# meyerls/PEGASUS

Measured on AMD Instinct MI355X. Metric: rendered views/sec (RGB+depth+mask) on 2M-Gaussian scene @800x800, higher is better.
Workload: dtype f32

## Files before the change

### pegasus_amd/csrc/cull.hip.h

```cpp
#pragma once
#include "pgr_common.h"

namespace pgr {

__device__ __forceinline__ float edge_min_q(float A, float B, float C, float r, float d_fixed, float lo, float hi) {
    float t = -(d_fixed * r);
    t = fminf(hi, fmaxf(lo, t));
    return A * d_fixed * d_fixed + 2.0f * B * d_fixed * t + C * t * t;
}

struct CullSplat { float mx, my, A, B, C, rBC, rBA, tau; uint32_t flags; };

__device__ __forceinline__ CullSplat make_cull_splat(float2 xy, float4 co, float rBC, float rBA) {
    CullSplat s;
    s.mx = xy.x; s.my = xy.y; s.A = co.x; s.B = co.y; s.C = co.z;
    s.flags = (co.w < ALPHA_MIN ? 1u : 0u)
            | ((!(co.x > 0.0f) || !(co.z > 0.0f)) ? 2u : 0u);
    s.rBC = rBC;
    s.rBA = rBA;
    const float t = 255.0f * co.w;
    const uint32_t bits = __float_as_uint(t);
    const float e = (float)((int)((bits >> 23) & 0xffu) - 127);
    const float m = __uint_as_float((bits & 0x007fffffu) | 0x3f800000u);
    s.tau = 1.3862944f * (e + (m - 1.0f) + 0.0861f);
    return s;
}

__device__ __forceinline__ CullSplat make_cull_splat(float2 xy, float4 co) {
    return make_cull_splat(xy, co, co.y / co.z, co.y / co.x);
}

__device__ __forceinline__ bool rect_may_contribute(const CullSplat& s, float x0, float y0, float x1, float y1) {
    if (s.flags & 1u) return false;
    if (s.flags & 2u) return true;
    if (s.mx >= x0 && s.mx <= x1 && s.my >= y0 && s.my <= y1) return true;
    const float dx0 = x0 - s.mx, dx1 = x1 - s.mx, dy0 = y0 - s.my, dy1 = y1 - s.my;
    const float dxn = s.mx < x0 ? dx0 : dx1, dyn = s.my < y0 ? dy0 : dy1;
    const float q = fminf(edge_min_q(s.A, s.B, s.C, s.rBC, dxn, dy0, dy1), edge_min_q(s.C, s.B, s.A, s.rBA, dyn, dx0, dx1));
    const float DX = fmaxf(fabsf(dx0), fabsf(dx1)), DY = fmaxf(fabsf(dy0), fabsf(dy1));
    const float M = s.A * DX * DX + 2.0f * fabsf(s.B) * DX * DY + s.C * DY * DY;
    return !(q > s.tau + 0.00001f * M + 0.01f);
}

__device__ __forceinline__ bool tile_may_contribute(const CullSplat& s, int tx, int ty, int W, int H) {
    const float x0 = (float)(tx * TILE), y0 = (float)(ty * TILE);
    const float x1 = fminf(x0 + (float)(TILE - 1), (float)(W - 1));
    const float y1 = fminf(y0 + (float)(TILE - 1), (float)(H - 1));
    return rect_may_contribute(s, x0, y0, x1, y1);
}


}
```

### pegasus_amd/csrc/tilebin.hip.h

```cpp
#pragma once
#include <type_traits>

#include "composite.hip.h"
#include "cull.hip.h"
#include "pgr_common.h"

namespace pgr {

constexpr int BIN_CHUNK = 4096;
#ifndef PGR_BIN_THREADS
#define PGR_BIN_THREADS 512
#endif
constexpr int BIN_THREADS = PGR_BIN_THREADS;
constexpr int BIN_LDS_TILES = 16384;
constexpr int SORT_THREADS = 256;

__device__ __forceinline__ uint2 pack_rect(int minx, int miny, int maxx, int maxy) {
    return make_uint2((uint32_t)minx | ((uint32_t)miny << 16), (uint32_t)maxx | ((uint32_t)maxy << 16));
}

struct BinView {
    const uint2* rects;
    const float4* splats;
    uint32_t* tile_count;
    uint32_t* rel;
    uint2* ranges;
    uint32_t* counters;
    uint2* bucket;
    uint32_t* gauss_sorted;
    uint64_t* alt;
    uint32_t* obj_last;
    int32_t n_env;
    const int32_t* tie_index;
    const uint32_t* tie_inv;
    uint2* records;
};


__device__ __forceinline__ uint32_t dpp_u32(uint32_t old, uint32_t v, int ctrl, int row_mask, bool bound) {
    switch (ctrl) {
        case 0x111: return (uint32_t)__builtin_amdgcn_update_dpp((int)old, (int)v, 0x111, 0xF, 0xF, true);
        case 0x112: return (uint32_t)__builtin_amdgcn_update_dpp((int)old, (int)v, 0x112, 0xF, 0xF, true);
        case 0x114: return (uint32_t)__builtin_amdgcn_update_dpp((int)old, (int)v, 0x114, 0xF, 0xF, true);
        case 0x118: return (uint32_t)__builtin_amdgcn_update_dpp((int)old, (int)v, 0x118, 0xF, 0xF, true);
        case 0x142: return (uint32_t)__builtin_amdgcn_update_dpp((int)old, (int)v, 0x142, 0xA, 0xF, false);
        default:    return (uint32_t)__builtin_amdgcn_update_dpp((int)old, (int)v, 0x143, 0xC, 0xF, false);
    }
}

__device__ __forceinline__ uint32_t wave_inclusive_scan(uint32_t v) {
    v += dpp_u32(0, v, 0x111, 0xF, true);
    v += dpp_u32(0, v, 0x112, 0xF, true);
    v += dpp_u32(0, v, 0x114, 0xF, true);
    v += dpp_u32(0, v, 0x118, 0xF, true);
    v += dpp_u32(0, v, 0x142, 0xA, false);
    v += dpp_u32(0, v, 0x143, 0xC, false);
    return v;
}

__device__ __forceinline__ uint32_t wave_inclusive_max(uint32_t v) {
    v = max(v, dpp_u32(0, v, 0x111, 0xF, true));
    v = max(v, dpp_u32(0, v, 0x112, 0xF, true));
    v = max(v, dpp_u32(0, v, 0x114, 0xF, true));
    v = max(v, dpp_u32(0, v, 0x118, 0xF, true));
    v = max(v, dpp_u32(0, v, 0x142, 0xA, false));
    v = max(v, dpp_u32(0, v, 0x143, 0xC, false));
    return v;
}

constexpr int BIN_STAGE_WORDS = WAVE * 12 + WAVE;
constexpr int BIN_THREADS_SMALL = 1024;
__host__ __device__ inline size_t bin_lds_bytes(int tiles, int threads) {
    return ((size_t)(tiles < BIN_LDS_TILES ? tiles : BIN_LDS_TILES) + 3) / 4 * 16 + (size_t)(threads / WAVE) * BIN_STAGE_WORDS * 4 + 16;
}

struct BinLayers {
    const int32_t* layer_id;
    int32_t layer_tiles;
    int32_t layer_rows;
    int32_t n_layers;
};
constexpr uint32_t VERDICT_WINDOWS = 62;
constexpr uint32_t VERDICT_REGION_WORDS = 192;

template <bool SCATTER, int THREADS>
__global__ __launch_bounds__(THREADS) void bin_kernel(const BinView* __restrict__ views, int n, int grid_x,
                                                          int tiles, int W, int H, const uint32_t* __restrict__ vis,
                                                          int vis_words, int verdict_groups,
                                                          BinLayers layers = BinLayers{nullptr, 0, 0, 0}) {
    extern __shared__ __attribute__((aligned(16))) uint32_t lds[];
    constexpr int BIN_WAVES = THREADS / WAVE;
    const BinView& bv = views[blockIdx.y];
    if (SCATTER && gload(bv.counters + 1)) return;
    const int chunk = blockIdx.x;
    const int begin = chunk * BIN_CHUNK, end = min(n, begin + BIN_CHUNK);
    const int lane = threadIdx.x & (WAVE - 1), wave = threadIdx.x / WAVE;
    const bool layered = layers.layer_id != nullptr;
    const int hist_words = (min(layered ? layers.layer_tiles : tiles, BIN_LDS_TILES) + 3) / 4 * 4;
    float4* const stage = reinterpret_cast<float4*>(lds + hist_words + wave * BIN_STAGE_WORDS);
    uint32_t* const heads = reinterpret_cast<uint32_t*>(stage + WAVE * 3);
    uint32_t* const ctrl = lds + hist_words + BIN_WAVES * BIN_STAGE_WORDS;
    constexpr int GROUPS = BIN_CHUNK / WAVE;
    static_assert(GROUPS == WAVE, "one visibility bit per lane of a wave");
    int pass_first = 0, pass_last = (tiles - 1) / BIN_LDS_TILES;
    if (layered) {
        if (begin >= end) return;
        pass_first = max(1, min(layers.n_layers + 1, (int)gload(layers.layer_id + begin)));
        pass_last = min(layers.n_layers, (int)gload(layers.layer_id + end - 1));
    }
    for (int lp = pass_first; lp <= pass_last; ++lp) {
        const int lo = layered ? (lp - 1) * layers.layer_tiles : lp * BIN_LDS_TILES;
        const int span = layered ? layers.layer_tiles : min(BIN_LDS_TILES, tiles - lo);
        const int row_off = layered ? (lp - 1) * layers.layer_rows : 0;
        for (int t = threadIdx.x; t < span; t += THREADS)
            lds[t] = SCATTER ? gload(bv.ranges + lo + t).x + gload(bv.rel + (size_t)chunk * tiles + lo + t) : 0u;
        if (wave == 0) {
            const int b = begin + lane * WAVE;
            bool visible = b < end;
            if (visible && vis) visible = (vis[(size_t)(b / WAVE) * vis_words + (blockIdx.y >> 5)] >> (blockIdx.y & 31)) & 1u;
            const uint64_t m = __ballot(visible);
            if (lane == 0) { ctrl[0] = 0u; ctrl[1] = (uint32_t)m; ctrl[2] = (uint32_t)(m >> 32); }
        }
        __syncthreads();
        const uint64_t vis_bits = ((uint64_t)ctrl[2] << 32) | ctrl[1];
        auto take_ticket = [&]() {
            for (;;) {
                uint32_t ticket = 0;
                if (lane == 0) ticket = atomicAdd(&ctrl[0], 1u);
                ticket = (uint32_t)__builtin_amdgcn_readfirstlane((int)ticket);
                if (ticket >= (uint32_t)GROUPS || ((vis_bits >> ticket) & 1ull)) return ticket;
            }
        };
        for (uint32_t ticket = take_ticket(); ticket < (uint32_t)GROUPS; ticket = take_ticket()) {
            const int base = begin + (int)ticket * WAVE;
            bool has_region = base / WAVE < verdict_groups;
            if (layered) {
                const int l0 = gload(layers.layer_id + base), l1 = gload(layers.layer_id + min(base + WAVE, end) - 1);
                if (lp < l0 || lp > l1) continue;
                has_region = has_region && l0 == l1;
            }
            uint32_t* const region = reinterpret_cast<uint32_t*>(bv.records) + (size_t)(base / WAVE) * VERDICT_REGION_WORDS;
            uint64_t* const ballots = reinterpret_cast<uint64_t*>(region + WAVE);
            const int i = base + lane;
            const int ic = i < end ? i : end - 1;
            uint2 r = gload(bv.rects + ic);
            float4 q0 = make_float4(0.f, 0.f, 0.f, 0.f), q1 = q0;
            float depth = 0.0f;
            uint64_t my_ballot = 0;
            if (SCATTER && has_region) {
                depth = __uint_as_float(gload(region + lane));
                if (lane < (int)VERDICT_WINDOWS) my_ballot = gload(ballots + lane);
            } else {
                q0 = gload(bv.splats + (size_t)ic * 3);
                q1 = gload(bv.splats + (size_t)ic * 3 + 1);
                if (SCATTER || has_region) depth = gload(reinterpret_cast<const float*>(bv.splats + (size_t)ic * 3 + 2) + 3);
            }
            if (i >= end) r = make_uint2(0u, 0u);
            const int w = (int)(r.y & 0xffff) - (int)(r.x & 0xffff), h = (int)(r.y >> 16) - (int)(r.x >> 16);
            const uint32_t area = (w > 0 && h > 0) ? (uint32_t)(w * h) : 0u;
            const uint32_t incl = wave_inclusive_scan(area);
            const uint32_t excl = incl - area;
            const uint32_t total = (uint32_t)__builtin_amdgcn_readlane((int)incl, WAVE - 1);
            const bool bits = has_region && total <= VERDICT_WINDOWS * (uint32_t)WAVE;
            if (SCATTER && has_region && !bits) {
                q0 = gload(bv.splats + (size_t)ic * 3);
                q1 = gload(bv.splats + (size_t)ic * 3 + 1);
                depth = gload(reinterpret_cast<const float*>(bv.splats + (size_t)ic * 3 + 2) + 3);
            }
            auto walk = [&](auto from_bits_c, auto write_bits_c) {
                constexpr bool FROM_BITS = decltype(from_bits_c)::value, WRITE_BITS = decltype(write_bits_c)::value;
                float4 s0 = make_float4(0.f, 0.f, 0.f, 0.f), s1 = s0, s2 = s0;
                if (area) {
                    uint32_t flags = 0;
                    if (!FROM_BITS) {
                        const CullSplat cs = make_cull_splat(make_float2(q0.x, q0.y), make_float4(q0.z, q0.w, q1.x, q1.y), q1.z, q1.w);
                        s0 = make_float4(cs.mx, cs.my, cs.A, cs.B);
                        s1 = make_float4(cs.C, cs.rBC, cs.rBA, cs.tau);
                        flags = cs.flags;
                    }
                    s2 = make_float4(__uint_as_float(flags | ((uint32_t)w << 2)), __uint_as_float(r.x), 1.0f / (float)w, depth);
                }
                if (!FROM_BITS) { stage[lane * 3 + 0] = s0; stage[lane * 3 + 1] = s1; }
                stage[lane * 3 + 2] = s2;
                __builtin_amdgcn_wave_barrier();
                if (WRITE_BITS && total) gstore(region + lane, __float_as_uint(depth));
                uint32_t carry_key = 0;
                uint32_t it = 0;
                for (uint32_t c0 = 0; c0 < total; c0 += WAVE, ++it) {
                    uint64_t verdicts = ~0ull;
                    if (FROM_BITS) {
                        const uint32_t vlo = (uint32_t)__builtin_amdgcn_readlane((int)(uint32_t)my_ballot, (int)it);
                        const uint32_t vhi = (uint32_t)__builtin_amdgcn_readlane((int)(uint32_t)(my_ballot >> 32), (int)it);
                        verdicts = ((uint64_t)vhi << 32) | vlo;
                    }
                    heads[lane] = 0u;
                    asm volatile("" ::: "memory");
                    if (area && excl - c0 < (uint32_t)WAVE) heads[excl - c0] = ((excl + 1u) << 6) | (uint32_t)lane;
                    asm volatile("" ::: "memory");
                    uint32_t key = wave_inclusive_max(heads[lane]);
                    asm volatile("" ::: "memory");
                    key = key ? key : carry_key;
                    carry_key = (uint32_t)__builtin_amdgcn_readlane((int)key, WAVE - 1);
                    if (FROM_BITS && verdicts == 0ull) continue;
                    const uint32_t c = c0 + (uint32_t)lane;
                    const int g = (int)(key & 63u);
                    const uint32_t k = c - ((key >> 6) - 1u);
                    const float4 o2 = stage[g * 3 + 2];
                    const uint32_t fw = __float_as_uint(o2.x), rlo = __float_as_uint(o2.y);
                    const int ow = (int)(fw >> 2);
                    int ty = (int)(((float)k + 0.5f) * o2.z);
                    int tx = (int)k - ty * ow;
                    if (tx < 0) { --ty; tx += ow; } else if (tx >= ow) { ++ty; tx -= ow; }
                    const int x = (int)(rlo & 0xffff) + tx, y = (int)(rlo >> 16) + ty;
                    const int t = y * grid_x + x - lo;
                    bool pass = c < total && (unsigned)t < (unsigned)span;
                    if (FROM_BITS) {
                        pass = pass && ((verdicts >> lane) & 1ull);
                    } else if (pass) {
                        const float4 o0 = stage[g * 3 + 0], o1 = stage[g * 3 + 1];
                        CullSplat cs;
                        cs.mx = o0.x; cs.my = o0.y; cs.A = o0.z; cs.B = o0.w;
                        cs.C = o1.x; cs.rBC = o1.y; cs.rBA = o1.z; cs.tau = o1.w; cs.flags = fw & 3u;
                        pass = tile_may_contribute(cs, x, y - row_off, W, H);
                    }
                    if (WRITE_BITS) {
                        const uint64_t m = __ballot(pass);
                        if (lane == 0) gstore(ballots + it, m);
                    }
                    if (pass) {
                        const uint32_t slot = atomicAdd(&lds[t], 1u);
                        if (SCATTER) gstore(bv.bucket + slot, make_uint2(__float_as_uint(o2.w), (uint32_t)(base + g)));
                    }
                }
            };
            if (SCATTER) {
                if (bits) walk(std::true_type{}, std::false_type{}); else walk(std::false_type{}, std::false_type{});
            } else {
                if (bits) walk(std::false_type{}, std::true_type{}); else walk(std::false_type{}, std::false_type{});
            }
        }
        __syncthreads();
        if (!SCATTER) {
            for (int t = threadIdx.x; t < span; t += THREADS) {
                const uint32_t cnt = lds[t];
                gstore(bv.rel + (size_t)chunk * tiles + lo + t, cnt ? gatomic_add(bv.tile_count + lo + t, cnt) : 0u);
            }
            __syncthreads();
        }
    }
}

__global__ void invert_tie_index_kernel(int n, const int32_t* __restrict__ tie_index, uint32_t* __restrict__ tie_inv) {
    const int i = blockIdx.x * blockDim.x + threadIdx.x;
    if (i >= n) return;
    const int k = tie_index[i];
    if ((unsigned)k < (unsigned)n) tie_inv[k] = (uint32_t)i;
}

__global__ __launch_bounds__(1024) void tile_scan_kernel(const BinView* __restrict__ views, int tiles,
                                                         uint32_t max_instances, int grid_x,
                                                         uint32_t* __restrict__ order_state, int skip_empty,
                                                         uint32_t* __restrict__ host_status) {
    __shared__ unsigned long long wave_tot[1024 / WAVE];
    __shared__ unsigned long long carry_s;
    __shared__ uint32_t hist[ORDER_BINS];
    __shared__ uint32_t last_s;
    const BinView& bv = views[blockIdx.x];
    const int lane = threadIdx.x & (WAVE - 1), wid = threadIdx.x / WAVE;
    if (threadIdx.x == 0) carry_s = 0;
    if (threadIdx.x < ORDER_BINS) hist[threadIdx.x] = 0;
    __syncthreads();
    for (int base = 0; base < tiles; base += 1024) {
        const int idx = base + threadIdx.x;
        const unsigned long long v = idx < tiles ? (unsigned long long)bv.tile_count[idx] : 0ull;
        unsigned long long s = v;
#pragma unroll
        for (int d = 1; d < WAVE; d <<= 1) {
            const unsigned long long t = __shfl_up(s, d, WAVE);
            if (lane >= d) s += t;
        }
        if (lane == WAVE - 1) wave_tot[wid] = s;
        __syncthreads();
        unsigned long long wave_prefix = 0;
        for (int w = 0; w < wid; ++w) wave_prefix += wave_tot[w];
        const unsigned long long carry = carry_s;
        const unsigned long long excl = carry + wave_prefix + s - v;
        const unsigned long long cap = max_instances;
        if (idx < tiles) {
            const uint2 r = make_uint2((uint32_t)min(excl, cap), (uint32_t)min(excl + v, cap));
            bv.ranges[idx] = r;
            if (order_state && !(skip_empty && r.y == r.x))
                atomicAdd(&hist[xcd_of_tile(idx, grid_x) * ORDER_CLASSES_USED + coarse_class(r.y - r.x)], ITEMS_PER_TILE);
        }
        __syncthreads();
        if (threadIdx.x == 1023) carry_s = carry + wave_prefix + s;
        __syncthreads();
    }
    if (threadIdx.x == 0) {
        const uint32_t total = (uint32_t)min(carry_s, 0xffffffffull);
        const uint32_t over = carry_s > (unsigned long long)max_instances ? 1u : 0u;
        bv.counters[0] = total;
        bv.counters[1] = over;
        if (host_status) {
            host_status[2 * blockIdx.x] = total;
            host_status[2 * blockIdx.x + 1] = over;
            __threadfence_system();
        }
    }
    if (!order_state) return;
    if (gridDim.x == 1) {
        __syncthreads();
        if (threadIdx.x < NUM_XCD) {
            uint32_t acc = 0;
            for (int c = 0; c < ORDER_CLASSES_USED; ++c) {
                gstore(order_state + threadIdx.x * ORDER_CLASSES_USED + c, acc);
                acc += hist[threadIdx.x * ORDER_CLASSES_USED + c];
            }
        }
        return;
    }
    if (threadIdx.x < ORDER_BINS && hist[threadIdx.x]) gatomic_add(order_state + threadIdx.x, hist[threadIdx.x]);
    __threadfence();
    __syncthreads();
    if (threadIdx.x == 0) last_s = gatomic_add(order_state + ORDER_DONE_WORD, 1u) == gridDim.x - 1u ? 1u : 0u;
    __syncthreads();
    if (!last_s) return;
    __threadfence();
    if (threadIdx.x < NUM_XCD) {
        uint32_t acc = 0;
        for (int c = 0; c < ORDER_CLASSES_USED; ++c) {
            const uint32_t v = gatomic_load(order_state + threadIdx.x * ORDER_CLASSES_USED + c);
            gstore(order_state + threadIdx.x * ORDER_CLASSES_USED + c, acc);
            acc += v;
        }
    }
}


constexpr uint64_t KEY_INF = ~0ull;

__device__ __forceinline__ uint32_t key_to_pos(const uint32_t* __restrict__ inv, uint32_t tk) { return inv ? gload(inv + tk) : tk; }

template <int E>
__device__ __forceinline__ void register_sort(uint64_t (&r)[E]) {
#pragma unroll
    for (int k = 2; k <= E; k <<= 1) {
#pragma unroll
        for (int i = 0; i < E; ++i) {
            const int j = i ^ (k - 1);
            if (j > i) {
                const uint64_t a = r[i], b = r[j];
                const bool sw = a > b;
                r[i] = sw ? b : a;
                r[j] = sw ? a : b;
            }
        }
#pragma unroll
        for (int s = k >> 2; s >= 1; s >>= 1) {
#pragma unroll
            for (int i = 0; i < E; ++i) {
                const int j = i ^ s;
                if (j > i) {
                    const uint64_t a = r[i], b = r[j];
                    const bool sw = a > b;
                    r[i] = sw ? b : a;
                    r[j] = sw ? a : b;
                }
            }
        }
    }
}

template <int E>
__device__ __forceinline__ int pad_idx(int i) {
    return i + i / E;
}

template <int THREADS, typename Get>
__device__ __forceinline__ void mark_last_object(Get get, int n, int n_env, uint32_t* __restrict__ obj_last,
                                                 uint32_t pos_offset = 0) {
    uint32_t best = 0;
    for (int i = threadIdx.x; i < n; i += THREADS)
        if ((int)get(i) >= n_env) best = pos_offset + (uint32_t)i + 1u;
#pragma unroll
    for (int m = 1; m < WAVE; m <<= 1) best = max(best, (uint32_t)__shfl_xor((int)best, m));
    if ((threadIdx.x & (WAVE - 1)) == 0 && best) gatomic_max(obj_last, best);
}

template <int THREADS, int E>
__device__ __forceinline__ void merge_sort_tile(uint64_t* __restrict__ skeys, const uint2* __restrict__ bucket,
                                                uint32_t* __restrict__ out, int n, uint64_t* keys_out = nullptr,
                                                int n_env = -1, uint32_t* __restrict__ obj_last = nullptr,
                                                uint32_t pos_offset = 0, const int32_t* __restrict__ tie = nullptr,
                                                const uint32_t* __restrict__ inv = nullptr) {
    const int t = threadIdx.x;
    uint64_t r[E];
#pragma unroll
    for (int e = 0; e < E; ++e) {
        const int i = e * THREADS + t;
        uint64_t k = KEY_INF;
        if (i < n) {
            const uint2 v = gload(bucket + i);
            k = ((uint64_t)v.x << 32) | (tie ? (uint32_t)gload(tie + v.y) : v.y);
        }
        r[e] = k;
    }
    register_sort<E>(r);
#pragma unroll
    for (int e = 0; e < E; ++e) skeys[t * (E + 1) + e] = r[e];
    __syncthreads();

    const int total = THREADS * E;
    for (int run = E; run < total; run <<= 1) {
        const int o_glob = t * E;
        const int a0 = o_glob & ~(2 * run - 1), b0 = a0 + run;
        const int o = o_glob - a0;
        int lo = o > run ? o - run : 0, hi = o < run ? o : run;
        while (lo < hi) {
            const int mid = (lo + hi + 1) >> 1;
            const uint64_t a = skeys[pad_idx<E>(a0 + mid - 1)];
            const uint64_t b = skeys[pad_idx<E>(b0 + o - mid)];
            if (a <= b) lo = mid; else hi = mid - 1;
        }
        int i = lo, j = o - lo;
        uint64_t av = i < run ? skeys[pad_idx<E>(a0 + i)] : KEY_INF;
        uint64_t bv = j < run ? skeys[pad_idx<E>(b0 + j)] : KEY_INF;
#pragma unroll
        for (int e = 0; e < E; ++e) {
            const bool takeA = (j >= run) || (i < run && av <= bv);
            r[e] = takeA ? av : bv;
            if (takeA) { ++i; av = i < run ? skeys[pad_idx<E>(a0 + i)] : KEY_INF; }
            else       { ++j; bv = j < run ? skeys[pad_idx<E>(b0 + j)] : KEY_INF; }
        }
        __syncthreads();
#pragma unroll
        for (int e = 0; e < E; ++e) skeys[t * (E + 1) + e] = r[e];
        __syncthreads();
    }
    if (keys_out) {
        for (int i = t; i < n; i += THREADS) gstore(keys_out + i, skeys[pad_idx<E>(i)]);
    } else {
        for (int i = t; i < n; i += THREADS) gstore(out + i, key_to_pos(inv, (uint32_t)skeys[pad_idx<E>(i)]));
        if (n_env >= 0)
            mark_last_object<THREADS>([&](int i) { return key_to_pos(inv, (uint32_t)skeys[pad_idx<E>(i)]); }, n, n_env, obj_last,
                                      pos_offset);
    }
}


constexpr uint32_t BUCKET_SQ_LIMIT = 8;

constexpr int SORT_MISC_BYTES = 256;

template <int THREADS, int E, int NB = THREADS * E, int KEYS = THREADS * E>
__device__ __forceinline__ bool bucket_sort_tile(unsigned char* __restrict__ lds, const uint2* __restrict__ bucket,
                                                     uint32_t* __restrict__ out, int n, int n_env,
                                                     uint32_t* __restrict__ obj_last, uint32_t pos_offset = 0,
                                                     const int32_t* __restrict__ tie = nullptr) {
    constexpr int CAP = THREADS * E, WAVES = THREADS / WAVE, CH = NB / (WAVES * WAVE);
    static_assert(NB % (WAVES * WAVE) == 0, "bucket count");
    static_assert(4 * WAVES * 4 <= SORT_MISC_BYTES, "per-wave words must fit the bytes the callers reserve behind the counters");
    static_assert(KEYS <= CAP, "key image");
    uint64_t* s_keys = reinterpret_cast<uint64_t*>(lds);
    uint32_t* s_hist = reinterpret_cast<uint32_t*>(lds + (size_t)KEYS * 8);
    uint32_t* s_wmin = s_hist + NB;
    uint32_t* s_wmax = s_wmin + WAVES;
    uint32_t* s_wtot = s_wmax + WAVES;
    uint32_t* s_wsq = s_wtot + WAVES;
    const int t = threadIdx.x, lane = t & (WAVE - 1), wave = t / WAVE;

    uint32_t d[E], id[E];
    uint32_t dmin = 0xffffffffu, dmax = 0u;
    {
        uint2 v[E];
#pragma unroll
        for (int e = 0; e < E; ++e) v[e] = gload(bucket + min(e * THREADS + t, n - 1));
        for (int i = t; i < NB; i += THREADS) s_hist[i] = 0u;
#pragma unroll
        for (int e = 0; e < E; ++e) {
            const bool in = e * THREADS + t < n;
            d[e] = in ? v[e].x : 0xffffffffu; id[e] = in ? v[e].y : 0xffffffffu;
            dmin = min(dmin, d[e]); dmax = max(dmax, in ? v[e].x : 0u);
        }
    }
    dmin = ~wave_inclusive_max(~dmin);
    dmax = wave_inclusive_max(dmax);
    if (lane == WAVE - 1) { s_wmin[wave] = dmin; s_wmax[wave] = dmax; }
    __syncthreads();
    uint32_t mn = 0xffffffffu, mx = 0u;
#pragma unroll
    for (int w = 0; w < WAVES; ++w) { mn = min(mn, s_wmin[w]); mx = max(mx, s_wmax[w]); }
    const float scale = (float)NB / ((float)(mx - mn) + 1.0f);
    auto bucket_of = [&](uint32_t depth) { return min((uint32_t)((float)(depth - mn) * scale), (uint32_t)(NB - 1)); };
    uint32_t br[E];
#pragma unroll
    for (int e = 0; e < E; ++e) {
        br[e] = 0u;
        if (e * THREADS + t < n) {
            const uint32_t b = bucket_of(d[e]);
            br[e] = (b << 16) | atomicAdd(&s_hist[b], 1u);
        }
    }
    __syncthreads();
    const int wbase = wave * (WAVE * CH);
    constexpr bool KEEP_H = E <= 8;
    uint32_t h[KEEP_H ? CH : 1];
    uint32_t tot = 0, sq = 0;
#pragma unroll
    for (int c = 0; c < CH; ++c) {
        const uint32_t hc = s_hist[wbase + c * WAVE + lane];
        if (KEEP_H) h[c] = hc;
        tot += hc; sq += hc * hc;
    }
    tot = wave_inclusive_scan(tot);
    sq = wave_inclusive_scan(sq);
    if (lane == WAVE - 1) { s_wtot[wave] = tot; s_wsq[wave] = sq; }
    __syncthreads();
    uint32_t carry = 0, sqsum = 0;
#pragma unroll
    for (int w = 0; w < WAVES; ++w) {
        const uint32_t tw = s_wtot[w];
        carry += w < wave ? tw : 0u;
        sqsum += s_wsq[w];
    }
    if (sqsum > BUCKET_SQ_LIMIT * (uint32_t)n * (uint32_t)((CAP + NB - 1) / NB)) { __syncthreads(); return false; }
#pragma unroll
    for (int c = 0; c < CH; ++c) {
        const uint32_t hc = KEEP_H ? h[c] : s_hist[wbase + c * WAVE + lane];
        const uint32_t incl = wave_inclusive_scan(hc);
        s_hist[wbase + c * WAVE + lane] = (carry + incl - hc) | (hc << 16);
        carry += (uint32_t)__builtin_amdgcn_readlane((int)incl, WAVE - 1);
    }
    __syncthreads();
#pragma unroll
    for (int e = 0; e < E; ++e)
        if (e * THREADS + t < n)
            s_keys[(s_hist[br[e] >> 16] & 0xffffu) + (br[e] & 0xffffu)] = ((uint64_t)d[e] << 32) | id[e];
    __syncthreads();
    constexpr int EB = E < 8 ? E : 8;
    uint32_t best = 0;
#pragma unroll
// ... 654 lines not shown
```

Before: 6123.

## Process two tile candidates per lane in count pass using packed f32x2 culling

In the non-scatter (counting) bin pass, each loop iteration now handles two 64-candidate windows per lane. Tile culling for the pair runs through packed f32x2 arithmetic, and the head-scan staging buffer is doubled to 2*WAVE. The goal is to halve loop trips and scan overhead and to use packed FP32 math for the cull test. In exchange it raises register pressure and LDS staging size, and it writes two ballot words per iteration.

```diff
diff --git a/pegasus_amd/csrc/cull.hip.h b/pegasus_amd/csrc/cull.hip.h
--- a/pegasus_amd/csrc/cull.hip.h
+++ b/pegasus_amd/csrc/cull.hip.h
@@ -49,5 +49,41 @@
     return rect_may_contribute(s, x0, y0, x1, y1);
 }
 
+__device__ __forceinline__ f32x2_t edge_min_q2(f32x2_t A, f32x2_t B, f32x2_t C, f32x2_t r, f32x2_t d_fixed, f32x2_t lo, f32x2_t hi) {
+    f32x2_t t = -(d_fixed * r);
+    t.x = fminf(hi.x, fmaxf(lo.x, t.x));
+    t.y = fminf(hi.y, fmaxf(lo.y, t.y));
+    return A * d_fixed * d_fixed + 2.0f * B * d_fixed * t + C * t * t;
+}
+
+struct CullSplat2 { f32x2_t mx, my, A, B, C, rBC, rBA, tau; uint32_t flags[2]; };
+
+__device__ __forceinline__ void rect_may_contribute2(const CullSplat2& s, f32x2_t x0, f32x2_t y0, f32x2_t x1, f32x2_t y1,
+                                                     bool& keep0, bool& keep1) {
+    const f32x2_t dx0 = x0 - s.mx, dx1 = x1 - s.mx, dy0 = y0 - s.my, dy1 = y1 - s.my;
+    f32x2_t dxn, dyn, DX, DY, aB;
+    dxn.x = s.mx.x < x0.x ? dx0.x : dx1.x; dxn.y = s.mx.y < x0.y ? dx0.y : dx1.y;
+    dyn.x = s.my.x < y0.x ? dy0.x : dy1.x; dyn.y = s.my.y < y0.y ? dy0.y : dy1.y;
+    const f32x2_t qx = edge_min_q2(s.A, s.B, s.C, s.rBC, dxn, dy0, dy1), qy = edge_min_q2(s.C, s.B, s.A, s.rBA, dyn, dx0, dx1);
+    DX.x = fmaxf(fabsf(dx0.x), fabsf(dx1.x)); DX.y = fmaxf(fabsf(dx0.y), fabsf(dx1.y));
+    DY.x = fmaxf(fabsf(dy0.x), fabsf(dy1.x)); DY.y = fmaxf(fabsf(dy0.y), fabsf(dy1.y));
+    aB.x = fabsf(s.B.x); aB.y = fabsf(s.B.y);
+    const f32x2_t M = s.A * DX * DX + 2.0f * aB * DX * DY + s.C * DY * DY;
+    const f32x2_t bound = s.tau + 0.00001f * M + 0.01f;
+    const bool in0 = s.mx.x >= x0.x && s.mx.x <= x1.x && s.my.x >= y0.x && s.my.x <= y1.x;
+    const bool in1 = s.mx.y >= x0.y && s.mx.y <= x1.y && s.my.y >= y0.y && s.my.y <= y1.y;
+    keep0 = !(s.flags[0] & 1u) && ((s.flags[0] & 2u) || in0 || !(fminf(qx.x, qy.x) > bound.x));
+    keep1 = !(s.flags[1] & 1u) && ((s.flags[1] & 2u) || in1 || !(fminf(qx.y, qy.y) > bound.y));
+}
+
+__device__ __forceinline__ void tile_may_contribute2(const CullSplat2& s, int tx0, int ty0, int tx1, int ty1, int W, int H,
+                                                     bool& keep0, bool& keep1) {
+    const f32x2_t x0 = {(float)(tx0 * TILE), (float)(tx1 * TILE)}, y0 = {(float)(ty0 * TILE), (float)(ty1 * TILE)};
+    const f32x2_t xe = x0 + (float)(TILE - 1), ye = y0 + (float)(TILE - 1);
+    const f32x2_t x1 = {fminf(xe.x, (float)(W - 1)), fminf(xe.y, (float)(W - 1))};
+    const f32x2_t y1 = {fminf(ye.x, (float)(H - 1)), fminf(ye.y, (float)(H - 1))};
+    rect_may_contribute2(s, x0, y0, x1, y1, keep0, keep1);
+}
+
 
 }
diff --git a/pegasus_amd/csrc/tilebin.hip.h b/pegasus_amd/csrc/tilebin.hip.h
--- a/pegasus_amd/csrc/tilebin.hip.h
+++ b/pegasus_amd/csrc/tilebin.hip.h
@@ -68,7 +68,7 @@
     return v;
 }
 
-constexpr int BIN_STAGE_WORDS = WAVE * 12 + WAVE;
+constexpr int BIN_STAGE_WORDS = WAVE * 12 + 2 * WAVE;
 constexpr int BIN_THREADS_SMALL = 1024;
 __host__ __device__ inline size_t bin_lds_bytes(int tiles, int threads) {
     return ((size_t)(tiles < BIN_LDS_TILES ? tiles : BIN_LDS_TILES) + 3) / 4 * 16 + (size_t)(threads / WAVE) * BIN_STAGE_WORDS * 4 + 16;
@@ -167,8 +167,8 @@
                 q1 = gload(bv.splats + (size_t)ic * 3 + 1);
                 depth = gload(reinterpret_cast<const float*>(bv.splats + (size_t)ic * 3 + 2) + 3);
             }
-            auto walk = [&](auto from_bits_c, auto write_bits_c) {
-                constexpr bool FROM_BITS = decltype(from_bits_c)::value, WRITE_BITS = decltype(write_bits_c)::value;
+            auto walk = [&](auto from_bits_c) {
+                constexpr bool FROM_BITS = decltype(from_bits_c)::value;
                 float4 s0 = make_float4(0.f, 0.f, 0.f, 0.f), s1 = s0, s2 = s0;
                 if (area) {
                     uint32_t flags = 0;
@@ -183,7 +183,6 @@
                 if (!FROM_BITS) { stage[lane * 3 + 0] = s0; stage[lane * 3 + 1] = s1; }
                 stage[lane * 3 + 2] = s2;
                 __builtin_amdgcn_wave_barrier();
-                if (WRITE_BITS && total) gstore(region + lane, __float_as_uint(depth));
                 uint32_t carry_key = 0;
                 uint32_t it = 0;
                 for (uint32_t c0 = 0; c0 < total; c0 += WAVE, ++it) {
@@ -223,20 +222,80 @@
                         cs.C = o1.x; cs.rBC = o1.y; cs.rBA = o1.z; cs.tau = o1.w; cs.flags = fw & 3u;
                         pass = tile_may_contribute(cs, x, y - row_off, W, H);
                     }
-                    if (WRITE_BITS) {
-                        const uint64_t m = __ballot(pass);
-                        if (lane == 0) gstore(ballots + it, m);
-                    }
                     if (pass) {
                         const uint32_t slot = atomicAdd(&lds[t], 1u);
-                        if (SCATTER) gstore(bv.bucket + slot, make_uint2(__float_as_uint(o2.w), (uint32_t)(base + g)));
+                        gstore(bv.bucket + slot, make_uint2(__float_as_uint(o2.w), (uint32_t)(base + g)));
                     }
                 }
             };
-            if (SCATTER) {
-                if (bits) walk(std::true_type{}, std::false_type{}); else walk(std::false_type{}, std::false_type{});
+            auto walk_pair = [&](auto write_bits_c) {
+                constexpr bool WRITE_BITS = decltype(write_bits_c)::value;
+                float4 s0 = make_float4(0.f, 0.f, 0.f, 0.f), s1 = s0, s2 = s0;
+                if (area) {
+                    const CullSplat cs = make_cull_splat(make_float2(q0.x, q0.y), make_float4(q0.z, q0.w, q1.x, q1.y), q1.z, q1.w);
+                    s0 = make_float4(cs.mx, cs.my, cs.A, cs.B);
+                    s1 = make_float4(cs.C, cs.rBC, cs.rBA, cs.tau);
+                    s2 = make_float4(__uint_as_float(cs.flags | ((uint32_t)w << 2)), __uint_as_float(r.x), 1.0f / (float)w, depth);
+                }
+                stage[lane * 3 + 0] = s0; stage[lane * 3 + 1] = s1; stage[lane * 3 + 2] = s2;
+                __builtin_amdgcn_wave_barrier();
+                if (WRITE_BITS && total) gstore(region + lane, __float_as_uint(depth));
+                uint32_t carry_key = 0;
+                uint32_t it = 0;
+                for (uint32_t c0 = 0; c0 < total; c0 += 2 * WAVE, it += 2) {
+                    heads[lane] = 0u; heads[WAVE + lane] = 0u;
+                    asm volatile("" ::: "memory");
+                    if (area && excl - c0 < 2u * WAVE) heads[excl - c0] = ((excl + 1u) << 6) | (uint32_t)lane;
+                    asm volatile("" ::: "memory");
+                    const uint32_t h0 = heads[lane], h1 = heads[WAVE + lane];
+                    asm volatile("" ::: "memory");
+                    uint32_t key0 = wave_inclusive_max(h0), key1 = wave_inclusive_max(h1);
+                    key0 = key0 ? key0 : carry_key;
+                    key1 = key1 ? key1 : (uint32_t)__builtin_amdgcn_readlane((int)key0, WAVE - 1);
+                    carry_key = (uint32_t)__builtin_amdgcn_readlane((int)key1, WAVE - 1);
+                    const uint32_t ca = c0 + (uint32_t)lane, cb = ca + (uint32_t)WAVE;
+                    const int ga = (int)(key0 & 63u), gb = (int)(key1 & 63u);
+                    const uint32_t ka = ca - ((key0 >> 6) - 1u), kb = cb - ((key1 >> 6) - 1u);
+                    const float4 oa = stage[ga * 3 + 2], ob = stage[gb * 3 + 2];
+                    const uint32_t fwa = __float_as_uint(oa.x), fwb = __float_as_uint(ob.x);
+                    const uint32_t rla = __float_as_uint(oa.y), rlb = __float_as_uint(ob.y);
+                    const int owa = (int)(fwa >> 2), owb = (int)(fwb >> 2);
+                    const f32x2_t tyf = ((f32x2_t){(float)ka, (float)kb} + 0.5f) * (f32x2_t){oa.z, ob.z};
+                    int tya = (int)tyf.x, tyb = (int)tyf.y;
+                    int txa = (int)ka - tya * owa, txb = (int)kb - tyb * owb;
+                    if (txa < 0) { --tya; txa += owa; } else if (txa >= owa) { ++tya; txa -= owa; }
+                    if (txb < 0) { --tyb; txb += owb; } else if (txb >= owb) { ++tyb; txb -= owb; }
+                    const int xa = (int)(rla & 0xffff) + txa, ya = (int)(rla >> 16) + tya;
+                    const int xb = (int)(rlb & 0xffff) + txb, yb = (int)(rlb >> 16) + tyb;
+                    const int ta = ya * grid_x + xa - lo, tb = yb * grid_x + xb - lo;
+                    bool pa = ca < total && (unsigned)ta < (unsigned)span;
+                    bool pb = cb < total && (unsigned)tb < (unsigned)span;
+                    if (pa || pb) {
+                        const float4 a0 = stage[ga * 3 + 0], a1 = stage[ga * 3 + 1];
+                        const float4 b0 = stage[gb * 3 + 0], b1 = stage[gb * 3 + 1];
+                        CullSplat2 cs;
+                        cs.mx = (f32x2_t){a0.x, b0.x}; cs.my = (f32x2_t){a0.y, b0.y};
+                        cs.A = (f32x2_t){a0.z, b0.z}; cs.B = (f32x2_t){a0.w, b0.w};
+                        cs.C = (f32x2_t){a1.x, b1.x}; cs.rBC = (f32x2_t){a1.y, b1.y};
+                        cs.rBA = (f32x2_t){a1.z, b1.z}; cs.tau = (f32x2_t){a1.w, b1.w};
+                        cs.flags[0] = fwa & 3u; cs.flags[1] = fwb & 3u;
+                        bool keep_a, keep_b;
+                        tile_may_contribute2(cs, xa, ya - row_off, xb, yb - row_off, W, H, keep_a, keep_b);
+                        pa = pa && keep_a;
+                        pb = pb && keep_b;
+                    }
+                    if (WRITE_BITS) {
+                        const uint64_t ma = __ballot(pa), mb = __ballot(pb);
+                        if (lane < (c0 + (uint32_t)WAVE < total ? 2 : 1)) gstore(ballots + it + lane, lane ? mb : ma);
+                    }
+                    if (pa) atomicAdd(&lds[ta], 1u);
+                    if (pb) atomicAdd(&lds[tb], 1u);
+                }
+            };
+            if constexpr (SCATTER) {
+                if (bits) walk(std::true_type{}); else walk(std::false_type{});
             } else {
-                if (bits) walk(std::false_type{}, std::true_type{}); else walk(std::false_type{}, std::false_type{});
+                if (bits) walk_pair(std::true_type{}); else walk_pair(std::false_type{});
             }
         }
         __syncthreads();
```

Measured after the change: 5860. 0.957x the previous value.
